# 10183308/popsift

Measured on AMD Instinct MI355X. Metric: Mpix/s SIFT extract on 1920x1080 (keypoints+descriptors), higher is better.
Workload: dtype f32; 1 GPU; 1920x1080 u8 grayscale, default popsift::Config (2x upscale, 9 octaves, 3 levels, PopSift mode, loop descriptor, RootSift); distinct_images_per_gpu=16, contexts_per_gpu=3, images_per_launch=16

## Files before the change

popsift_amd/csrc/ctx.hip:

```cpp
#include <hip/hip_runtime.h>

#include <algorithm>
#include <atomic>
#include <cmath>
#include <cstdarg>
#include <cstddef>
#include <cstdio>
#include <cstdlib>
#include <cstring>
#include <new>
#include <type_traits>
#include <vector>

#include "devfeatures.h"
#include "kernels.h"
#include "sift_types.h"
#include "trace.h"

using namespace popsift_hip;

namespace {

constexpr int PITCH_ALIGN = 64;
constexpr int PROFILE_REPS = 4;

template <int N>
struct GaussRows {
    float filter[N * PS_GA];
    int   span[N];
    float sigma[N];
};

struct EventPair {
    hipEvent_t a, b;
    double     bytes;
    bool       big;
};

template <class T, size_t PER = 1>
struct DevBuf {
    T*     p = nullptr;
    size_t cap = 0;
    hipError_t release()
    {
        const hipError_t e = p ? hipFree(p) : hipSuccess;
        if (e == hipSuccess) {
            p = nullptr;
            cap = 0;
        }
        return e;
    }
};

}

struct ImageSlot {
    DevBuf<char> input;
    void*        h_input = nullptr;
    size_t       h_input_cap = 0;
    DevBuf<float>       arena;
    DevBuf<InitExt>     iext;
    DevBuf<InitExt>     iext2;
    DevBuf<FilterState> fstate;
    DevBuf<int>         fhist;
    DevBuf<InitExt>     otmp;
    DevBuf<int>         orows;
    DevBuf<Ext>         ext;
    DevBuf<float, PS_ORI_NBINS> ohist;
    DevBuf<popsift_hip_feature> feats;
    DevBuf<float, 128> desc;
    DevBuf<int>        map;
    DevBuf<float2>     rot;
    DevBuf<DescRec>    drec;
    DevBuf<int2>       cand;
    DevBuf<int>        partial;
    DevBuf<int>        ovf;
    bool               sized = false;
    DevBuf<popsift_hip_feature> alt_feats;
    DevBuf<float, 128>          alt_desc;
    bool moved = false;
    DevBuf<uint8_t, 128> desc_u8;
    bool u8_read = false;
    DevBuf<popsift_hip_frame>   frames;
    popsift_hip_frame*          h_frames = nullptr;
    DevBuf<int>                 fcounts, perm, inv;
    DevBuf<popsift_hip_feature> lfeats;
    int n_frames = 0;

    size_t desc_cap() const { return std::min({desc.cap, map.cap, rot.cap, drec.cap}); }

    void release()
    {
        auto each = [](auto&... b) { ((void)b.release(), ...); };
        each(input, arena, iext, iext2, fstate, fhist, otmp, orows, ext, ohist, feats, desc, map, rot, drec, cand, partial, ovf, alt_feats,
             alt_desc, desc_u8, frames, fcounts, perm, inv, lfeats);
        if (h_input) (void)hipHostFree(h_input);
        if (h_frames) (void)hipHostFree(h_frames);
    }
};

struct popsift_hip_ctx {
    int                device = 0;
    popsift_hip_params p{};
    int                levels = 3, L = 6;
    GaussRows<POPSIFT_HIP_MAX_LEVELS> tab{};
    GaussRows<POPSIFT_HIP_MAX_LEVELS> abs0{};
    float*             d_abs0 = nullptr;
    int                direct_path = 0;
    GaussRows<POPSIFT_HIP_MAX_OCTAVES> dd{};
    float*             d_dd = nullptr;
    int                scale_path = 0;
    SiftConsts         sc{};
    hipStream_t        stream = nullptr;
    hipEvent_t         ev_begin = nullptr, ev_end = nullptr;
    hipEvent_t         ev_stage[POPSIFT_HIP_STAGE_COUNT + 1] = {};

    int  in_w = 0, in_h = 0;
    int  frozen_octaves = -1;
    bool have_image = false, finished = false;
    bool batch_ok = false;
    int  nb = 1;
    bool describe = false;
    int  ori_given = 0;
    int  frames_max = 0;

    ImageSlot slot[PS_MAX_BATCH];
    BatchDesc bd{};
    PyrDesc   pd{};
    int       kp_waves = 65536;
    int       det_qcap = 1 << 30;
    int       desc_rows = 1 << 30;
    int       desc_list = 1 << 30;
    BlurTune  blur_tune{0, 0};
    int       order_coarse = 0;
    int       pyr_tail = 0;
    int       cand_cap_init = 1 << 20;
    bool      cand_cap_user = false;
    int       ohist_cap_init = 0;
    int       desc_cap_init = 0;
    size_t    ext_cap = 0;
    int       cand_cap = 0, desc_cap = 0;
    size_t    ohist_cap = 0;
    hipStream_t copy_stream = nullptr;
    hipEvent_t  ev_u8 = nullptr;
    bool     copy_pending = false;
    unsigned long submit_seq = 0, copy_seq = 0;
    Counters* d_ct = nullptr;
    Counters* h_ct = nullptr;
    PyrDesc*  d_pd = nullptr;
    PyrDesc*  h_pd = nullptr;
    int       n_feat[PS_MAX_BATCH] = {}, n_desc[PS_MAX_BATCH] = {};

    int                    fail_alloc_in = 0;
    int                    profile = 0;
    std::vector<EventPair> blur_events;
    size_t                 blur_events_used = 0;
    popsift_hip_report     rep{};

    char err[256] = {0};
};

namespace {

int fail(popsift_hip_ctx* c, int code, const char* fmt, ...)
{
    if (c) {
        va_list ap;
        va_start(ap, fmt);
        vsnprintf(c->err, sizeof(c->err), fmt, ap);
        va_end(ap);
    }
    return code;
}

#define HIP_TRY(c, call)                                                                              \
    do {                                                                                              \
        hipError_t e__ = (call);                                                                      \
// ... 102 lines not shown

void plan_dims(const popsift_hip_params& p, int w, int h, int octaves_cfg, int* n_oct, int* bw, int* bh)
{
    const float scaleFactor = 1.0f / powf(2.0f, -p.upscale_factor);
    int         oct = octaves_cfg;
    if (oct < 0) oct = std::max(int(floorf(logf((float)std::min(w, h)) / logf(2.0f)) - 3.0f + scaleFactor), 1);
    oct = std::min(oct, PS_MAX_OCT);
    *n_oct = oct;
    *bw = (int)ceilf(w * scaleFactor);
    *bh = (int)ceilf(h * scaleFactor);
}

const char* plan_pyramid(const popsift_hip_params& p, int levels, int L, int octaves_cfg, int w, int h, PyrDesc* out,
                         size_t* arena_floats, int* base_w, int* base_h)
{
    int n_oct, bw, bh;
    memset(out, 0, sizeof(*out));
    *arena_floats = 0;
    plan_dims(p, w, h, octaves_cfg, &n_oct, &bw, &bh);
    *base_w = bw;
    *base_h = bh;
    if (bw < 1 || bh < 1) return "scaled image is empty";
    if (bw > 32767 || bh > 32767) return "scaled image exceeds 32767 pixels per side";
    PyrDesc& pd = *out;
    size_t   total = 0;
    pd.n_oct = n_oct;
    pd.levels = levels;
    pd.L = L;
    pd.dog_fly = p.store_dog ? 0 : 1;
    int ow = bw, oh = bh, tiles = 0;
    for (int o = 0; o < n_oct; o++) {
        OctDesc& od = pd.o[o];
        od.w = ow;
        od.h = oh;
        od.pitch = (ow + PITCH_ALIGN - 1) / PITCH_ALIGN * PITCH_ALIGN;
        od.plane_stride = (int64_t)od.pitch * oh;
        od.tile_begin = tiles;
        tiles += extrema_units(ow, oh);
        od.data_off = (int64_t)total;
        total += (size_t)od.plane_stride * (size_t)L;
        if (!pd.dog_fly) {
            od.dog_off = (int64_t)total;
            total += (size_t)od.plane_stride * (size_t)(L - 1);
        }
        ow = (int)ceilf(ow / 2.0f);
        oh = (int)ceilf(oh / 2.0f);
    }
    if (pd.dog_fly) {
        for (int o = 0; o < n_oct; o++) pd.o[o].dog_off = (int64_t)total;
        total += (size_t)pd.o[0].plane_stride;
    }
    pd.total_tiles = tiles;
    *arena_floats = total;
    if (total * sizeof(float) >= ((size_t)1 << 32)) return "pyramid arena of 4 GiB or more: the image is too large";
    return nullptr;
}

hipError_t ctx_malloc(popsift_hip_ctx* c, void** p, size_t bytes)
{
    if (c->fail_alloc_in > 0 && --c->fail_alloc_in == 0) {
        *p = nullptr;
        return hipErrorOutOfMemory;
    }
    return hipMalloc(p, bytes);
}

template <class T, size_t PER>
int grow(popsift_hip_ctx* c, DevBuf<T, PER>& b, size_t need)
{
    if (need <= b.cap) return 0;
    HIP_TRY(c, b.release());
    HIP_TRY(c, ctx_malloc(c, (void**)&b.p, need * PER * sizeof(T)));
    b.cap = need;
    return 0;
}

void refresh_caps(popsift_hip_ctx* c)
{
    size_t cand = 1 << 30, desc = 1 << 30, hist = (size_t)1 << 40;
    for (int k = 0; k < c->nb; k++) {
        const ImageSlot& s = c->slot[k];
        cand = std::min(cand, s.cand.cap);
        desc = std::min(desc, s.desc_cap());
        hist = std::min(hist, s.ohist.cap);
        Slot& v = c->bd.s[k];
        v.arena = s.arena.p;
        v.ct = c->d_ct + k;
        v.cand = s.cand.p;
        v.ovf = s.ovf.p;
        v.iext = s.iext.p;
        v.iext2 = s.iext2.p;
        v.fstate = s.fstate.p;
        v.fhist = s.fhist.p;
        v.ohist = s.ohist.p;
        v.ext = s.ext.p;
        v.partial = s.partial.p;
        v.map = s.map.p;
        v.rot = s.rot.p;
        v.drec = s.drec.p;
        v.feats = s.feats.p;
        v.desc = s.desc.p;
    }
    c->cand_cap = (int)cand;
    c->desc_cap = (int)desc;
    c->ohist_cap = hist;
}

int slot_desc_cap(popsift_hip_ctx* c, ImageSlot& s, size_t need)
{
    if (need <= s.desc_cap()) return 0;
    HIP_TRY(c, s.desc.release());
    HIP_TRY(c, s.map.release());
    HIP_TRY(c, s.rot.release());
    HIP_TRY(c, s.drec.release());
    if (int rc = grow(c, s.desc, need)) return rc;
    if (int rc = grow(c, s.map, need)) return rc;
    if (int rc = grow(c, s.rot, need)) return rc;
    return grow(c, s.drec, need);
}

template <typename F>
int ensure_cap(popsift_hip_ctx* c, F grow_slot)
{
    int rc = 0;
    for (int k = 0; k < c->nb && !rc; k++) rc = grow_slot(c->slot[k]);
    refresh_caps(c);
    return rc;
}

int prepare_geometry(popsift_hip_ctx* c, int w, int h, int nb)
{
    const bool same = c->have_image && w == c->in_w && h == c->in_h && c->pd.n_oct > 0;
    PyrDesc    pd = c->pd;
    int        bw = c->rep.base_w, bh = c->rep.base_h;
    size_t     total = 0;
    if (!same) {
        PyrDesc plan;
        if (const char* why = plan_pyramid(c->p, c->levels, c->L, c->frozen_octaves, w, h, &plan, &total, &bw, &bh))
            return fail(c, POPSIFT_HIP_ERR_INVALID, why);
        if (c->sc.filter_max > 0 && !filter_supported(plan.n_oct, c->sc.max_extrema, c->sc.grid_size))
            return fail(c, POPSIFT_HIP_ERR_INVALID, "grid filter: grid size > 64 or octaves * max_extrema >= 2^25");
        c->frozen_octaves = plan.n_oct;

        c->in_w = c->in_h = 0;
        c->have_image = false;
        c->pd.n_oct = 0;
        c->ext_cap = 0;
        for (int k = 0; k < PS_MAX_BATCH; k++) c->slot[k].sized = false;

        pd = plan;
    } else {
        const OctDesc& last = pd.o[pd.n_oct - 1];
        total = pd.dog_fly ? (size_t)pd.o[0].dog_off + (size_t)pd.o[0].plane_stride
                           : (size_t)last.dog_off + (size_t)last.plane_stride * (size_t)(c->L - 1);
    }
    const size_t need_ext = (size_t)pd.n_oct * (size_t)c->sc.max_extrema;
    for (int k = 0; k < nb; k++) {
        ImageSlot& s = c->slot[k];
        if (s.sized) continue;
        if (int rc = grow(c, s.arena, total)) return rc;
        if (int rc = grow(c, s.iext, need_ext)) return rc;
        if (int rc = grow(c, s.ext, need_ext)) return rc;
        if (int rc = grow(c, s.feats, need_ext)) return rc;
        if (c->sc.filter_max > 0) {
            if (int rc = grow(c, s.iext2, need_ext)) return rc;
            if (int rc = grow(c, s.fstate, 1)) return rc;
            if (int rc = grow(c, s.fhist, filter_hist_bytes(c->sc.grid_size) / sizeof(int))) return rc;
        }
        if (c->p.feature_order == POPSIFT_HIP_ORDER_RASTER) {
            if (int rc = grow(c, s.otmp, need_ext)) return rc;
            if (int rc = grow(c, s.orows, order_rows(pd))) return rc;
        }
        if (int rc = grow(c, s.partial, (need_ext / scan_chunk() + 2) * scan_partials_per_chunk())) return rc;
        const int desc0 = c->desc_cap_init > 0 ? c->desc_cap_init
                                               : std::max(2 * c->sc.max_extrema, c->sc.max_extrema + c->sc.max_extrema / 4);
        if (int rc = slot_desc_cap(c, s, std::max(desc0, c->desc_cap))) return rc;
        int cand0 = std::max(c->cand_cap_init, DET_SUBQ);
        if (!c->cand_cap_user) {
            double px = 0;
            for (int o = 0; o < pd.n_oct; o++) px += (double)pd.o[o].w * pd.o[o].h;
            cand0 = std::max(cand0, (int)std::min(px / 8.0, 64.0 * 1024 * 1024));
        }
        if (int rc = grow(c, s.cand, std::max(cand0, c->cand_cap))) return rc;
        if (int rc = grow(c, s.ohist, std::max(c->ohist_cap_init > 0 ? (size_t)c->ohist_cap_init
                                                                      : std::min(need_ext, (size_t)2 * c->sc.max_extrema),
                                               c->slot[0].sized ? c->ohist_cap : (size_t)0)))
            return rc;
        if (int rc = grow(c, s.ovf, (size_t)pd.total_tiles + 1)) return rc;
        s.sized = true;
    }
    c->ext_cap = need_ext;
    if (!same) {
        *c->h_pd = pd;
        HIP_TRY(c, hipMemcpyAsync(c->d_pd, c->h_pd, sizeof(PyrDesc), hipMemcpyHostToDevice, c->stream));
        c->pd = pd;
        c->in_w = w;
        c->in_h = h;
        c->rep.num_octaves = pd.n_oct;
        c->rep.base_w = bw;
        c->rep.base_h = bh;
        double px = 0;
        for (int o = 0; o < pd.n_oct; o++) px += (double)pd.o[o].w * pd.o[o].h;
        c->rep.pyramid_pixels = px;
    }
    return 0;
}

template <typename F>
int timed_launch(popsift_hip_ctx* c, double alg_bytes, const char* what, F launch, bool big = false)
{
    if (c->profile == 1) {
        if (c->blur_events_used == c->blur_events.size()) {
            EventPair ep;
            HIP_TRY(c, hipEventCreate(&ep.a));
            HIP_TRY(c, hipEventCreate(&ep.b));
            c->blur_events.push_back(ep);
        }
        EventPair& ep = c->blur_events[c->blur_events_used++];
        ep.bytes = alg_bytes * c->nb;
        ep.big = big;
        HIP_TRY(c, hipEventRecord(ep.a, c->stream));
        for (int rep = 0; rep < PROFILE_REPS; rep++) HIP_TRY(c, launch());
        HIP_TRY(c, hipEventRecord(ep.b, c->stream));
    } else {
        HIP_TRY(c, launch());
        SYNC_CHK(c, what);
    }
    (void)what;
    return 0;
}

int blur_launch(popsift_hip_ctx* c, const BlurArgs& a, int mode, int span, int tile_h, double alg_bytes)
{
    return timed_launch(
        c, alg_bytes, "k_blur_tile", [&] { return launch_blur(a, c->bd, c->nb, mode, span, tile_h, c->stream, c->blur_tune); },
        mode == 0 && tile_h == 64);
}

template <typename A>
void set_plane(A& a, const OctDesc& od, int tile_h)
{
    a.w = od.w;
    a.h = od.h;
    a.pitch = od.pitch;
    a.tiles_x = (od.w + blur_tile_w() - 1) / blur_tile_w();
    a.tiles_y = (od.h + tile_h - 1) / tile_h;
}

BlurArgs level_args(const popsift_hip_ctx* c, int o, int level)
{
    const PyrDesc& pd = c->pd;
    const OctDesc& od = pd.o[o];
    BlurArgs       a{};
    set_plane(a, od, blur_tile_h(od.w, od.h));
    memcpy(a.taps.g, &c->tab.filter[level * PS_GA], sizeof(a.taps.g));
    a.dst_off = od.data_off + level * od.plane_stride;
    a.src_off = od.data_off + (level - 1) * od.plane_stride;
    a.dog_off = pd.dog_fly ? -1 : od.dog_off + (level - 1) * od.plane_stride;
    a.next0_off = (level == pd.L - 3 && o + 1 < pd.n_oct) ? pd.o[o + 1].data_off : -1;
    a.next_pitch = (o + 1 < pd.n_oct) ? pd.o[o + 1].pitch : 0;
    return a;
}

float input_shift(const popsift_hip_ctx* c)
{
    if (c->p.sift_mode == POPSIFT_HIP_SIFT_POPSIFT || c->p.sift_mode == POPSIFT_HIP_SIFT_VLFEAT)
        return 0.5f * powf(2.0f, c->p.upscale_factor - 0);
// ... 356 lines not shown
        const size_t bytes = (size_t)w * h * esz;
        if (int rc = grow(c, s.input, bytes)) return rc;
        if (where == 2) {
            HIP_TRY(c, hipMemcpy2DAsync(s.input.p, (size_t)w * esz, imgs[k], (size_t)pitch * esz, (size_t)w * esz, (size_t)h,
                                        hipMemcpyHostToDevice, c->stream));
        } else {
            if (bytes > s.h_input_cap) {
                if (s.h_input) HIP_TRY(c, hipHostFree(s.h_input));
                s.h_input = nullptr;
                s.h_input_cap = 0;
                HIP_TRY(c, hipHostMalloc(&s.h_input, bytes, hipHostMallocDefault));
                s.h_input_cap = bytes;
            }
            for (int y = 0; y < h; y++)
                memcpy((char*)s.h_input + (size_t)y * w * esz, (const char*)imgs[k] + (size_t)y * pitch * esz, (size_t)w * esz);
            HIP_TRY(c, hipMemcpyAsync(s.input.p, s.h_input, bytes, hipMemcpyHostToDevice, c->stream));
        }
        c->bd.s[k].input = s.input.p;
        dpitch = w;
    }
    if (where != 1) aligned4 = (dpitch & 3) == 0;
    c->describe = da != nullptr;
    c->ori_given = da && da->ori_mode == POPSIFT_HIP_ORI_GIVEN;
    c->frames_max = 0;
    for (int k = 0; k < nb && da; k++) {
        ImageSlot& s = c->slot[k];
        if (int rc = prepare_frames(c, s)) return rc;
        const int nf = da->n_frames[k];
        s.n_frames = nf;
        c->frames_max = std::max(c->frames_max, nf);
        if (nf > 0) {
            memcpy(s.h_frames, da->frames[k], (size_t)nf * sizeof(popsift_hip_frame));
            HIP_TRY(c, hipMemcpyAsync(s.frames.p, s.h_frames, (size_t)nf * sizeof(popsift_hip_frame), hipMemcpyHostToDevice, c->stream));
        }
    }
    c->blur_events_used = 0;
    HIP_TRY(c, hipEventRecord(c->ev_begin, c->stream));
    if (c->profile == 2) HIP_TRY(c, hipEventRecord(c->ev_stage[POPSIFT_HIP_STAGE_PYRAMID], c->stream));
    if (int rc = enqueue_pyramid(c, is_f32, dpitch, aligned4)) return rc;
    if (int rc = da ? enqueue_describe_stages(c, true) : enqueue_keypoint_stages(c, true)) return rc;
    HIP_TRY(c, hipEventRecord(c->ev_end, c->stream));
    c->have_image = true;
    c->finished = false;
    c->batch_ok = true;
    c->submit_seq++;
    for (ImageSlot& sl : c->slot) sl.moved = false;
    return 0;
}

int finish(popsift_hip_ctx* c)
{
    if (!c->have_image || !c->batch_ok) return fail(c, POPSIFT_HIP_ERR_STATE, c->have_image ? "the last submit failed" : "no image submitted");
    if (c->finished) return 0;
    POPSIFT_RANGE("popsift_hip: wait");
    HIP_TRY(c, hipSetDevice(c->device));
    bool rerun = false, fits = false;
    for (int attempt = 0; attempt < 8; attempt++) {
        HIP_TRY(c, hipStreamSynchronize(c->stream));
        int  ori_max = 0, qmax = 0;
        long ext_max = 0;
        for (int k = 0; k < c->nb; k++) {
            const Counters& h = c->h_ct[k];
            ori_max = std::max(ori_max, h.ori_total);
            for (int q = 0; q < DET_SUBQ; q++) qmax = std::max(qmax, h.qcnt[q].n);
            long ext_sum = 0;
            for (int o = 0; o < c->pd.n_oct; o++) ext_sum += std::min(h.ext_ct[o], c->sc.max_extrema);
            ext_max = std::max(ext_max, ext_sum);
        }
        const bool desc_short = ori_max > c->desc_cap;
        const bool cand_short = qmax > c->cand_cap / DET_SUBQ;
        const bool hist_short = (size_t)ext_max > c->ohist_cap && !c->ori_given;
        if (!desc_short && !cand_short && !hist_short) {
            fits = true;
            break;
        }
        if (desc_short)
            if (int rc = ensure_cap(c, [&](ImageSlot& s) { return slot_desc_cap(c, s, ori_max + ori_max / 8 + 1024); }))
                return rc;
        if (cand_short)
            if (int rc = ensure_cap(c, [&](ImageSlot& s) { return grow(c, s.cand, DET_SUBQ * (qmax + qmax / 8 + 64)); }))
                return rc;
        if (hist_short) {
            const size_t need = (size_t)ext_max + (size_t)ext_max / 8 + 1024;
            if (int rc = ensure_cap(c, [&](ImageSlot& s) { return grow(c, s.ohist, need); })) return rc;
        }
        if (int rc = c->describe ? enqueue_describe_stages(c) : enqueue_keypoint_stages(c)) return rc;
        HIP_TRY(c, hipEventRecord(c->ev_end, c->stream));
        rerun = true;
    }
    if (!fits) return fail(c, POPSIFT_HIP_ERR_DEVICE, "the keypoint buffers still do not fit after 8 grow-and-rerun rounds");
    popsift_hip_report& r = c->rep;
    for (int k = 0; k < c->nb; k++) {
        c->n_feat[k] = c->describe ? c->slot[k].n_frames : c->h_ct[k].ext_total;
        c->n_desc[k] = std::min(c->h_ct[k].ori_total, c->desc_cap);
    }
    Counters& h0 = c->h_ct[0];
    int       next = h0.ori_total;
    for (int o = PS_MAX_OCT - 1; o >= 0; o--) {
        if (h0.ext_ct[o] > 0) {
            h0.ori_ct[o] = next - h0.ori_ps[o];
            next = h0.ori_ps[o];
        } else {
            h0.ori_ct[o] = 0;
            h0.ori_ps[o] = next;
        }
    }
    for (int o = 0; o < PS_MAX_OCT; o++) {
        r.ext_ct[o] = h0.ext_ct[o];
        r.ori_ct[o] = h0.ori_ct[o];
    }
    r.ext_total = c->h_ct[0].ext_total;
    r.ori_total = c->n_desc[0];
    float ms = 0.0f;
    if (hipEventElapsedTime(&ms, c->ev_begin, c->ev_end) == hipSuccess) r.ms_device = ms;
    for (int k = 0; k < 8; k++) r.ms_stage[k] = 0.0f;
    if (c->profile == 2 && !rerun)
        for (int k = 0; k < POPSIFT_HIP_STAGE_COUNT; k++) {
            float t = 0.0f;
            if (hipEventElapsedTime(&t, c->ev_stage[k], c->ev_stage[k + 1]) == hipSuccess) r.ms_stage[k] = t;
        }
    r.ms_blur = 0.0f;
    r.blur_launches = 0;
    r.blur_alg_bytes = 0.0;
    r.ms_big = 0.0f;
    r.big_launches = 0;
    r.big_alg_bytes = 0.0;
    for (size_t i = 0; i < c->blur_events_used; i++) {
        float t = 0.0f;
        if (hipEventElapsedTime(&t, c->blur_events[i].a, c->blur_events[i].b) == hipSuccess) {
            t /= (float)PROFILE_REPS;
            r.ms_blur += t;
            r.blur_launches++;
            r.blur_alg_bytes += c->blur_events[i].bytes;
            if (c->blur_events[i].big) {
                r.ms_big += t;
                r.big_launches++;
                r.big_alg_bytes += c->blur_events[i].bytes;
            }
        }
    }
    c->finished = true;
    return 0;
}

int drain_copy(popsift_hip_ctx* c)
{
    if (!c->copy_pending) return 0;
    c->copy_pending = false;
    HIP_TRY(c, hipStreamSynchronize(c->copy_stream));
    return 0;
}

int results_here(popsift_hip_ctx* c, int k = 0)
{
    if (int rc = finish(c)) return rc;
    if (k < 0 || k >= c->nb) return fail(c, POPSIFT_HIP_ERR_INVALID, "the batch has %d images", c->nb);
    if (c->slot[k].moved)
        return fail(c, POPSIFT_HIP_ERR_STATE, "the results of this image were handed to popsift_hip_fetch_begin");
    return 0;
}

int slot_u8_ready(popsift_hip_ctx* c, ImageSlot& sl)
{
    if (sl.u8_read && c->copy_pending) HIP_TRY(c, hipStreamSynchronize(c->copy_stream));
    sl.u8_read = false;
    return grow(c, sl.desc_u8, std::max<size_t>(sl.desc_cap(), 1));
}
// ... 1278 lines not shown
```

popsift_amd/csrc/keypoint.hip:

```cpp
#include <hip/hip_runtime.h>

#include "kernels.h"
#include "sift_types.h"

namespace popsift_hip {
namespace {

constexpr float F_PI = 3.14159265358979323846f;
constexpr float F_PI2 = 2.0f * 3.14159265358979323846f;
constexpr float            ORI_WINFACTOR = 1.5f;
constexpr float            DESC_MAGNIFY = 3.0f;

typedef unsigned long long fix64;
__device__ __forceinline__ fix64 to_fix(float w) { return (fix64)(unsigned int)(w * 1048576.0f); }
__device__ __forceinline__ float from_fix(fix64 v) { return (float)((double)v * (1.0 / 1048576.0)); }


__device__ __forceinline__ void wave_lds_sync()
{
    __builtin_amdgcn_fence(__ATOMIC_SEQ_CST, "wavefront");
    __builtin_amdgcn_wave_barrier();
}

__device__ __forceinline__ int wave_incl_scan(int v)
// ... 120 lines not shown
    r = (ay > ax) ? 1.5707963267948966f - r : r;
    r = (x < 0.0f) ? 3.14159265358979323846f - r : r;
    return (y < 0.0f) ? -r : r;
}

__device__ __forceinline__ void sincos_cr(float ang, float& s, float& c)
{
    const double x = (double)ang;
    const double q = rint(x * 0.63661977236758134308);
    double       r = fma(-q, 1.57079632679489655800e+00, x);
    r = fma(-q, 6.12323399573676603587e-17, r);
    const double z = r * r;
    double       ps = 2.81145725434552075980e-15;
    ps = fma(ps, z, -7.64716373181981647590e-13);
    ps = fma(ps, z, 1.60590438368216145994e-10);
    ps = fma(ps, z, -2.50521083854417187751e-08);
    ps = fma(ps, z, 2.75573192239858906526e-06);
    ps = fma(ps, z, -1.98412698412698412698e-04);
    ps = fma(ps, z, 8.33333333333333333333e-03);
    ps = fma(ps, z, -1.66666666666666666667e-01);
    const double sr = fma(ps * z, r, r);
    double       pc = -1.56192069685862264622e-16;
    pc = fma(pc, z, 4.77947733238738529744e-14);
    pc = fma(pc, z, -1.14707455977297247139e-11);
    pc = fma(pc, z, 2.08767569878680989792e-09);
    pc = fma(pc, z, -2.75573192239858906526e-07);
    pc = fma(pc, z, 2.48015873015873015873e-05);
    pc = fma(pc, z, -1.38888888888888888889e-03);
    pc = fma(pc, z, 4.16666666666666666667e-02);
    pc = fma(pc, z, -0.5);
    const double cr = fma(pc, z, 1.0);
    const int    n = (int)q & 3;
    const double sd = (n & 1) ? cr : sr, cd = (n & 1) ? sr : cr;
    s = (float)((n & 2) ? -sd : sd);
    c = (float)(((n + 1) & 2) ? -cd : cd);
}

__device__ __forceinline__ float octants(float t, float x, float y, float ax, float ay)
{
    const unsigned int sgn = 0x80000000u;
    const float a = __uint_as_float(__float_as_uint(1.0f - t) ^ (__float_as_uint(ax - ay) & sgn));
    const float b = __uint_as_float(__float_as_uint(1.0f + a) ^ (__float_as_uint(x) & sgn));
    return copysignf(2.0f - b, y);
}

__device__ __forceinline__ float atan2_bins(float y, float x)
{
    const float ax = fabsf(x), ay = fabsf(y);
    const float mx = fmaxf(fmaxf(ax, ay), 1e-30f), mn = fminf(ax, ay);
    const float r = mn * __builtin_amdgcn_rcpf(mx);
    const float s = r * r;
    float       p = fmaf(-0.01492126751691103f, s, 0.06703268736600876f);
    p = fmaf(p, s, -0.14823880791664124f);
    p = fmaf(p, s, 0.24642325937747955f);
    p = fmaf(p, s, -0.42350852489471436f);
    p = fmaf(p, s, 1.2732105255126953f);
    return octants(p * r, x, y, ax, ay);
}

__device__ __forceinline__ float atan2_bins9(float y, float x)
{
    const float ax = fabsf(x), ay = fabsf(y);
    const float mx = fmaxf(fmaxf(ax, ay), 1e-30f), mn = fminf(ax, ay);
    const float r = mn * __builtin_amdgcn_rcpf(mx);
    const float s = r * r;
    float       p = fmaf(0.026540832594037056f, s, -0.1084246039390564f);
    p = fmaf(p, s, 0.22938621044158936f);
    p = fmaf(p, s, -0.4205572307109833f);
    p = fmaf(p, s, 1.2730693817138672f);
    return octants(p * r, x, y, ax, ay);
}

typedef float v2f __attribute__((ext_vector_type(2)));
typedef __attribute__((address_space(3))) fix64 lds_fix64;
typedef __attribute__((address_space(3))) unsigned int lds_u32;
typedef __attribute__((address_space(3))) short lds_i16;
typedef __attribute__((address_space(3))) unsigned long long lds_u64;

#ifndef KP_NW
#define KP_NW 1
#endif
constexpr int ORI_COPIES = 4;

__global__ __launch_bounds__(64 * KP_NW) void k_orientation(const PyrDesc* __restrict__ pdp, BatchDesc bd, SiftConsts sc,
                                                     int filtered, int hist_cap)
{
    const float* __restrict__   arena = bd.s[blockIdx.y].arena;
    Counters* __restrict__      ct = bd.s[blockIdx.y].ct;
    const InitExt* __restrict__ iext = filtered ? bd.s[blockIdx.y].iext2 : bd.s[blockIdx.y].iext;
    float* __restrict__         ohist = bd.s[blockIdx.y].ohist;
    const int n_oct = pdp->n_oct, L = pdp->L;
    constexpr int    NB = PS_ORI_NBINS + 2;
    __shared__ fix64 s_hist[KP_NW][ORI_COPIES][NB];
    const int        wave = threadIdx.x >> 6, lane = threadIdx.x & 63;
    fix64*           hall = &s_hist[wave][0][0];
    fix64*           hist = s_hist[wave][lane & (ORI_COPIES - 1)];

    __shared__ int ps[PS_MAX_OCT + 1];
    if (threadIdx.x == 0) ext_prefix(ct, sc, n_oct, ps);
    __syncthreads();
    const int total = min(ps[n_oct], hist_cap);

    for (XcdSlice sl = xcd_slice<KP_NW>(); sl.more(total); sl.s += sl.step) {
        const int g = sl.index();
        if (g >= total) continue;
        int o = 0;
        while (o + 1 < n_oct && g >= ps[o + 1]) o++;
        o = uniform(o);
        const InitExt  ie = iext[(size_t)o * sc.max_extrema + (g - uniform(ps[o]))];
        const OctDesc* od = &pdp->o[o];
        const int      w = uniform(od->w), h = uniform(od->h), pitch = uniform(od->pitch);
        const int      lvl = uniform(min(max(ie.lpos, 0), L - 1));
        const float*   layer = arena + uniform64(od->data_off + lvl * od->plane_stride);

        for (int k = lane; k < ORI_COPIES * NB; k += 64) hall[k] = 0ull;
        wave_lds_sync();

        const float x = uniformf(ie.xpos), y = uniformf(ie.ypos), sig = uniformf(ie.sigma);
        const float sigw = ORI_WINFACTOR * sig;
        const int   rad = (int)roundf(3.0f * sigw);
        const float factor2 = (-0.5f / (sigw * sigw)) * 1.4426950408889634f;
        const int   sq_thres = rad * rad;
        const int   xmin = max(1, (int)roundf(x) - rad);
        const int   xmax = min(w - 2, (int)roundf(x) + rad);
        const int   ymin = max(1, (int)roundf(y) - rad);
        const int   ymax = min(h - 2, (int)roundf(y) + rad);
        const int   wx = xmax - xmin + 1;
        const int   hy = ymax - ymin + 1;
#ifdef ORI_PROBE_NOLOOP
        const int   loops = 0;
#else
        const int   loops = (wx > 0 && hy > 0) ? wx * hy : 0;
#endif
        const float inv_wx = __builtin_amdgcn_rcpf((float)max(wx, 1));
        const float wxf = (float)wx, xminf = (float)xmin, yminf = (float)ymin, pitch4f = (float)(4 * pitch);
        const float* corner = layer + (size_t)(ymin * pitch + xmin);

        auto coord = [&](int i, float& fx, float& fy, unsigned int& off) {
            const float fi = (float)i;
            const float frow = floorf((fi + 0.5f) * inv_wx);
            const float fcol = fmaf(-frow, wxf, fi);
            fx = fcol + xminf;
            fy = frow + yminf;
            off = (unsigned int)fmaf(frow, pitch4f, fcol * 4.0f);
        };
        auto bin = [&](float fx, float fy, float gdx, float gdy, bool live) {
            const float dx = fx - x;
            const float dy = fy - y;
            const float sq_dist = truncf(dx * dx + dy * dy);
            if (live && sq_dist <= (float)sq_thres) {
                const float wfix = __builtin_amdgcn_sqrtf(fmaf(gdx, gdx, gdy * gdy)) * __builtin_amdgcn_exp2f(fmaf(sq_dist, factor2, 20.0f));
                float fb = fmaf(atan2_bins(gdy, gdx), (float)PS_ORI_NBINS / 8.0f, (float)PS_ORI_NBINS / 2.0f);
                if (fabsf((fb - floorf(fb)) - 0.5f) < 1e-4f) fb = (float)PS_ORI_NBINS * (atan2_acc(gdy, gdx) + F_PI) / F_PI2;
                int bidx;
                asm("v_cvt_rpi_i32_f32 %0, %1" : "=v"(bidx) : "v"(fb));
                atomicAdd(&hist[bidx], (fix64)(unsigned int)wfix);
            }
        };
        float        xa = 0.0f, ya = 0.0f, xb = 0.0f, yb = 0.0f;
        unsigned int oa = 0, ob = 0;
        float        a0 = 0.0f, a1 = 0.0f, a2 = 0.0f, a3 = 0.0f, b0 = 0.0f, b1 = 0.0f, b2 = 0.0f, b3 = 0.0f;
        const Taps   taps(corner, pitch);
        if (loops > 0) {
            coord(min(lane, loops - 1), xa, ya, oa);
            taps.load_b(oa, a0, a1, a2, a3);
        }
        for (int i = lane; i < loops; i += 128) {
            coord(min(i + 64, loops - 1), xb, yb, ob);
            taps.load_b(ob, b0, b1, b2, b3);
            bin(xa, ya, a0 - a1, a2 - a3, true);
            coord(min(i + 128, loops - 1), xa, ya, oa);
            taps.load_b(oa, a0, a1, a2, a3);
            bin(xb, yb, b0 - b1, b2 - b3, i + 64 < loops);
        }
        wave_lds_sync();

        if (lane < PS_ORI_NBINS) {
            fix64 acc = 0ull;
#pragma unroll
            for (int k = 0; k < ORI_COPIES; k++) acc += hall[k * NB + lane] + (lane == 0 ? hall[k * NB + PS_ORI_NBINS] : 0ull);
            ohist[(size_t)g * PS_ORI_NBINS + lane] = from_fix(acc);
        }
        wave_lds_sync();
    }
}

__device__ __forceinline__ float quad_from_prev(float v)
{
    return __int_as_float(__builtin_amdgcn_update_dpp(0, __float_as_int(v), 0x93, 0xf, 0xf, false));
}
__device__ __forceinline__ float quad_from_next(float v)
{
    return __int_as_float(__builtin_amdgcn_update_dpp(0, __float_as_int(v), 0x39, 0xf, 0xf, false));
}
template <int CTRL>
__device__ __forceinline__ int quad_xchg(int v)
{
    return __builtin_amdgcn_update_dpp(0, v, CTRL, 0xf, 0xf, false);
}
__device__ __forceinline__ float div3(float x)
{
    const float r = 0.333333343267440796f;
    const float q = x * r;
    return fmaf(fmaf(-3.0f, q, x), r, q);
}

__device__ __forceinline__ int ori_peaks_quad(const float* __restrict__ hsrc, int j, bool have, float* angle_out)
{
    constexpr int N = PS_ORI_NBINS, M = N / 4;
    float         h[M], t[M];
#pragma unroll
    for (int b = 0; b < M; b++) h[b] = have ? hsrc[M * j + b] : 0.0f;
#pragma unroll
    for (int pass = 0; pass < 3; pass++) {
        {
            const float lft = quad_from_prev(h[M - 1]), rgt = quad_from_next(h[0]);
#pragma unroll
            for (int b = 0; b < M; b++) t[b] = div3(((b == 0 ? lft : h[b - 1]) + h[b]) + (b == M - 1 ? rgt : h[b + 1]));
        }
        {
            const float lft = quad_from_prev(t[M - 1]), rgt = quad_from_next(t[0]);
#pragma unroll
            for (int b = 0; b < M; b++) h[b] = div3(((b == 0 ? lft : t[b - 1]) + t[b]) + (b == M - 1 ? rgt : t[b + 1]));
        }
    }
    float refined[M], yval[M];
    {
        const float lft = quad_from_prev(h[M - 1]), rgt = quad_from_next(h[0]);
#pragma unroll
        for (int b = 0; b < M; b++) {
            const int   bin = M * j + b;
            const int   prev = (bin == 0) ? N - 1 : bin - 1;
            const float hp = (b == 0) ? lft : h[b - 1], hv = h[b], hn = (b == M - 1) ? rgt : h[b + 1];
            bool        predicate = hv > fmaxf(hp, hn);
            const float num = predicate ? 3.0f * hp - 4.0f * hv + 1.0f * hn : 0.0f;
            const float denB = predicate ? 2.0f * (hp - 2.0f * hv + hn) : 1.0f;
            const float newbin = num / denB;
            predicate = (predicate && newbin >= 0.0f && newbin <= 2.0f);
            refined[b] = predicate ? prev + newbin : -1.0f;
            yval[b] = predicate ? -(num * num) / (4.0f * denB) + hp : -INFINITY;
        }
    }
    unsigned int used = 0u;
    float        best0 = 0.0f;
    int          angles = 0;
#pragma unroll
    for (int k = 0; k < POPSIFT_HIP_ORI_MAX; k++) {
        float bv = 0.0f, br = -1.0f;
        int   bi = -1;
#pragma unroll
        for (int b = 0; b < M; b++) {
            const bool take = !((used >> b) & 1u) && (bi < 0 || yval[b] > bv);
            bv = take ? yval[b] : bv;
            br = take ? refined[b] : br;
            bi = take ? M * j + b : bi;
        }
        {
// ... 733 lines not shown
                    }
                }
            } else
            for (int p = lane; p < 1600; p += 64) {
                const int   newy = p / 40, newx = p - newy * 40;
                const float stepx = stepbase + 0.125f * (float)newx;
                const float stepy = stepbase + 0.125f * (float)newy;
                const float ptx = cos_t * stepx + -sin_t * stepy;
                const float pty = cos_t * stepy + sin_t * stepx;
                const float px = x + ptx * SBP, py = y + pty * SBP;
                const float dxv = tex_linear(layer, width, height, pitch, px + cos_t, py + sin_t) -
                                  tex_linear(layer, width, height, pitch, px - cos_t, py - sin_t);
                const float dyv = tex_linear(layer, width, height, pitch, px - sin_t, py + cos_t) -
                                  tex_linear(layer, width, height, pitch, px + sin_t, py - cos_t);
                const float mod = __builtin_amdgcn_sqrtf(dxv * dxv + dyv * dyv);
                float       th = atan2_acc(dyv, dxv);
                th += (th < 0.0f ? F_PI2 : 0.0f);
                const float tth = th * M_4RPI;
                const float ffo = floorf(tth);
                const float do0 = tth - ffo;
                const int   b0 = (int)ffo & 7;
                const float ww = __expf(-0.125f * (stepx * stepx + stepy * stepy)) * mod * fscale;
                const float a1 = do0 * ww, a0 = ww - a1;
#pragma unroll
                for (int jy = 0; jy < 2; jy++) {
                    const int cy = (newy >> 3) - jy;
                    if (cy < 0 || cy > 3) continue;
                    const float wy = 1.0f - fabsf(-1.0f + 1.0f / 16.0f + 0.125f * (float)(newy - 8 * cy));
#pragma unroll
                    for (int jx = 0; jx < 2; jx++) {
                        const int cx = (newx >> 3) - jx;
                        if (cx < 0 || cx > 3) continue;
                        const float wx = 1.0f - fabsf(-1.0f + 1.0f / 16.0f + 0.125f * (float)(newx - 8 * cx));
                        const float wgt = wx * wy;
                        const unsigned int lo = (unsigned int)fmaf(a0, wgt, 0.5f);
                        const unsigned int hi = (unsigned int)fmaf(a1, wgt, 0.5f);
                        atomicAdd(&hist[((((cy << 2) + cx) << 3)) + b0], ((fix64)hi << 32) | lo);
                    }
                }
            }
        }
        wave_lds_sync();

        fix64     a0 = 0ull, a1 = 0ull;
        const int prevw = (lane & ~7) | ((lane + 7) & 7);
#pragma unroll
        for (int k = 0; k < DCOPY; k++) {
            a0 += (hall[k * 128 + lane] & 0xffffffffull) + (hall[k * 128 + prevw] >> 32);
            a1 += (hall[k * 128 + lane + 64] & 0xffffffffull) + (hall[k * 128 + prevw + 64] >> 32);
        }
        float v0 = (float)a0 * (1.0f / (float)(1 << FBITS)), v1 = (float)a1 * (1.0f / (float)(1 << FBITS));

        if (sc.norm_mode == POPSIFT_HIP_NORM_ROOTSIFT) {
            float sum = v0 + v1;
            sum = wave_allsum(sum);
            v0 = scalbnf(sqrtf(v0 / sum), sc.norm_multi);
            v1 = scalbnf(sqrtf(v1 / sum), sc.norm_multi);
        } else {
            float sq = v0 * v0 + v1 * v1;
            sq = wave_allsum(sq);
            const float norm = sqrtf(sq);
            v0 = fminf(v0, 0.2f * norm);
            v1 = fminf(v1, 0.2f * norm);
            sq = v0 * v0 + v1 * v1;
            sq = wave_allsum(sq);
            float rn = 1.0f / sqrtf(sq);
            rn = scalbnf(rn, sc.norm_multi);
            v0 = v0 * rn;
            v1 = v1 * rn;
        }
        desc[(size_t)d * 128 + lane] = v0;
        desc[(size_t)d * 128 + 64 + lane] = v1;
        wave_lds_sync();
    }
}



}

hipError_t launch_orientation(const PyrDesc* pd, const BatchDesc& bd, int nb, const SiftConsts& sc, bool filtered, int hist_cap,
                              int blocks, hipStream_t s)
{
    hipLaunchKernelGGL(k_orientation, dim3(blocks / KP_NW, nb), dim3(64 * KP_NW), 0, s, pd, bd, sc, filtered ? 1 : 0, hist_cap);
    return hipGetLastError();
}

hipError_t launch_scan(const PyrDesc* pd, const BatchDesc& bd, int nb, const SiftConsts& sc, bool filtered, int hist_cap,
                       int n_chunks, int desc_cap, hipStream_t s)
{
    hipLaunchKernelGGL(k_scan_local, dim3(std::min(n_chunks * SCAN_SUB, 512 * SCAN_SUB), nb), dim3(SCAN_LT), 0, s, pd, sc, bd,
                       filtered ? 1 : 0, hist_cap);
    hipLaunchKernelGGL(k_scan_apply, dim3(std::min(n_chunks, 1024), nb), dim3(256), 0, s, pd, sc, bd,
                       sc.desc_mode == POPSIFT_HIP_DESC_LOOP ? 1 : 0, desc_cap);
    return hipGetLastError();
}

hipError_t launch_scan_apply(const PyrDesc* pd, const BatchDesc& bd, int nb, const SiftConsts& sc, int n_chunks, int desc_cap,
                             hipStream_t s)
{
    hipLaunchKernelGGL(k_scan_apply, dim3(std::min(n_chunks, 1024), nb), dim3(256), 0, s, pd, sc, bd,
                       sc.desc_mode == POPSIFT_HIP_DESC_LOOP ? 1 : 0, desc_cap);
    return hipGetLastError();
}

int scan_chunk() { return SCAN_CHUNK; }
int scan_partials_per_chunk() { return SCAN_SUB; }

hipError_t launch_descriptors(const PyrDesc* pd, const BatchDesc& bd, int nb, const SiftConsts& sc, int desc_cap, int blocks,
                              hipStream_t s)
{
    if (sc.desc_mode == POPSIFT_HIP_DESC_NOTILE || sc.desc_mode == POPSIFT_HIP_DESC_IGRID)
        hipLaunchKernelGGL(k_descriptor_notile<false>, dim3(blocks / 4, nb), dim3(256), 0, s, pd, bd, sc, desc_cap);
    else if (sc.desc_mode == POPSIFT_HIP_DESC_ILOOP)
        hipLaunchKernelGGL(k_descriptor_notile<true>, dim3(blocks / 4, nb), dim3(256), 0, s, pd, bd, sc, desc_cap);
    else if (sc.desc_mode == POPSIFT_HIP_DESC_GRID)
        hipLaunchKernelGGL(k_descriptor_grid, dim3(blocks / 4, nb), dim3(256), 0, s, pd, bd, sc, desc_cap);
    else
        hipLaunchKernelGGL(k_descriptor, dim3(blocks / KP_NW, nb), dim3(64 * KP_NW), 0, s, bd, sc, desc_cap);
    return hipGetLastError();
}


}
```

popsift_amd/csrc/sift_types.h:

```cpp
#pragma once
#include <stdint.h>

#include <hip/hip_vector_types.h>

#include "../../include/popsift_hip.h"

#define PS_MAX_OCT POPSIFT_HIP_MAX_OCTAVES
#define PS_MAX_PLANES (POPSIFT_HIP_MAX_LEVELS + 3)
#define PS_GA POPSIFT_HIP_GAUSS_ALIGN
#define PS_ORI_NBINS 36

struct OctDesc {
    float*  data;
    float*  dog;
    int64_t data_off;
    int64_t dog_off;
    int64_t plane_stride;
    int     w, h, pitch;
    int     tile_begin;
};

struct PyrDesc {
    int     n_oct;
    int     levels;
    int     L;
    int     total_tiles;
    int     dog_fly;
    int     pad_;
    OctDesc o[PS_MAX_OCT];
};

struct SiftConsts {
    float sigma0, sigma_k, edge_limit, threshold;
    int   max_extrema, norm_multi, norm_mode, sift_mode;
    int   grid_size;
    int   up_fac_int;
    int   desc_mode;
    int   det_qcap;
    int   filter_max;
    int   filter_mode;
    int   desc_rows;
    int   desc_list;
};

struct InitExt {
    float xpos, ypos;
    int   lpos;
    float sigma;
    int   cell;
};

struct Ext {
    float xpos, ypos;
    int   lpos;
    float sigma;
    int   octave;
    int   num_ori;
    int   idx_ori;
    float orientation[POPSIFT_HIP_ORI_MAX];
};

struct DescRec {
    float        x, y;
    float        crsbp, srsbp;
    float        ang_bins;
    float        inv_c;
    unsigned int xymin, xymax;
    unsigned int off_lo, off_hi;
    unsigned int misc;
    float        inv_s;
};

static_assert(sizeof(DescRec) == 48, "three 16-byte loads");

struct Counters {
    int ext_ct[PS_MAX_OCT];
    int ori_ct[PS_MAX_OCT];
    int ext_ps[PS_MAX_OCT];
    int ori_ps[PS_MAX_OCT];
    int ext_total;
    int ori_total;
    int pad[2];
    struct {
        int n;
        int pad[31];
    } qcnt[64];
};
#define DET_SUBQ 64

#define PS_MAX_BATCH POPSIFT_HIP_MAX_BATCH
struct FilterState;
struct Slot {
    float*               arena;
    Counters*            ct;
    const void*          input;
    int2*                cand;
    int*                 ovf;
    InitExt*             iext;
    InitExt*             iext2;
    FilterState*         fstate;
    int*                 fhist;
    float*               ohist;
    Ext*                 ext;
    int*                 partial;
    int*                 map;
    float2*              rot;
    DescRec*             drec;
    popsift_hip_feature* feats;
    float*               desc;
};
struct BatchDesc {
    Slot s[PS_MAX_BATCH];
};

#define FILTER_MAX_CELLS 4096
struct FilterState {
    int                active;
    int                newlimit;
    int                pad[2];
    int                new_ct[PS_MAX_OCT];
    int                cell_count[FILTER_MAX_CELLS];
    int                cell_limit[FILTER_MAX_CELLS];
    int                remaining[FILTER_MAX_CELLS];
    int                cell_mode[FILTER_MAX_CELLS];
    unsigned long long prefix[FILTER_MAX_CELLS];
};

struct FrameSlot {
    const popsift_hip_frame* frames;
    int*                     counts;
    int*                     perm;
    int*                     inv;
    popsift_hip_feature*     lfeats;
    int                      n;
    int                      pad_;
};
struct FrameBatch {
    FrameSlot s[PS_MAX_BATCH];
};

struct OrderSlot {
    InitExt*        list;
    InitExt*        tmp;
    int*            rows;
    const Counters* ct;
};
struct OrderBatch {
    OrderSlot s[PS_MAX_BATCH];
};
struct OrderArgs {
    int n_oct, coarse, max_extrema;
    int chunks;
    int rows_total;
    int row_base[PS_MAX_OCT];
    int rows[PS_MAX_OCT];
};
```

Measured before the change: 3874 Mpix/s.

## Precompute per-keypoint orientation records in a prep kernel and restructure histogram loop

Adds a k_ori_prep kernel that computes each extremum's orientation window parameters (bounds, gaussian factor, threshold, corner offset) once per thread and stores them as 48-byte OriRec records. The orientation kernel then reads each record with three scalar 16-byte loads instead of doing the octave search, InitExt fetch and setup math per wave. It also splits the software-pipelined sample loop into a steady-state body with no bounds clamps and an explicit tail. This trades an extra kernel launch and an extra buffer write/read for less serial scalar setup in the wave-per-keypoint loop.

```diff
diff --git a/popsift_amd/csrc/ctx.hip b/popsift_amd/csrc/ctx.hip
--- a/popsift_amd/csrc/ctx.hip
+++ b/popsift_amd/csrc/ctx.hip
@@ -67,6 +67,7 @@
     DevBuf<int>         orows;
     DevBuf<Ext>         ext;
     DevBuf<float, PS_ORI_NBINS> ohist;
+    DevBuf<OriRec>              orec;
     DevBuf<popsift_hip_feature> feats;
     DevBuf<float, 128> desc;
     DevBuf<int>        map;
@@ -88,11 +89,12 @@
     int n_frames = 0;
 
     size_t desc_cap() const { return std::min({desc.cap, map.cap, rot.cap, drec.cap}); }
+    size_t hist_cap() const { return std::min(ohist.cap, orec.cap); }
 
     void release()
     {
         auto each = [](auto&... b) { ((void)b.release(), ...); };
-        each(input, arena, iext, iext2, fstate, fhist, otmp, orows, ext, ohist, feats, desc, map, rot, drec, cand, partial, ovf, alt_feats,
+        each(input, arena, iext, iext2, fstate, fhist, otmp, orows, ext, ohist, orec, feats, desc, map, rot, drec, cand, partial, ovf, alt_feats,
              alt_desc, desc_u8, frames, fcounts, perm, inv, lfeats);
         if (h_input) (void)hipHostFree(h_input);
         if (h_frames) (void)hipHostFree(h_frames);
@@ -361,7 +363,7 @@
         const ImageSlot& s = c->slot[k];
         cand = std::min(cand, s.cand.cap);
         desc = std::min(desc, s.desc_cap());
-        hist = std::min(hist, s.ohist.cap);
+        hist = std::min(hist, s.hist_cap());
         Slot& v = c->bd.s[k];
         v.arena = s.arena.p;
         v.ct = c->d_ct + k;
@@ -372,6 +374,7 @@
         v.fstate = s.fstate.p;
         v.fhist = s.fhist.p;
         v.ohist = s.ohist.p;
+        v.orec = s.orec.p;
         v.ext = s.ext.p;
         v.partial = s.partial.p;
         v.map = s.map.p;
@@ -396,6 +399,15 @@
     if (int rc = grow(c, s.map, need)) return rc;
     if (int rc = grow(c, s.rot, need)) return rc;
     return grow(c, s.drec, need);
+}
+
+int slot_hist_cap(popsift_hip_ctx* c, ImageSlot& s, size_t need)
+{
+    if (need <= s.hist_cap()) return 0;
+    HIP_TRY(c, s.ohist.release());
+    HIP_TRY(c, s.orec.release());
+    if (int rc = grow(c, s.ohist, need)) return rc;
+    return grow(c, s.orec, need);
 }
 
 template <typename F>
@@ -461,7 +473,7 @@
             cand0 = std::max(cand0, (int)std::min(px / 8.0, 64.0 * 1024 * 1024));
         }
         if (int rc = grow(c, s.cand, std::max(cand0, c->cand_cap))) return rc;
-        if (int rc = grow(c, s.ohist, std::max(c->ohist_cap_init > 0 ? (size_t)c->ohist_cap_init
+        if (int rc = slot_hist_cap(c, s, std::max(c->ohist_cap_init > 0 ? (size_t)c->ohist_cap_init
                                                                       : std::min(need_ext, (size_t)2 * c->sc.max_extrema),
                                                c->slot[0].sized ? c->ohist_cap : (size_t)0)))
             return rc;
@@ -984,7 +996,7 @@
                 return rc;
         if (hist_short) {
             const size_t need = (size_t)ext_max + (size_t)ext_max / 8 + 1024;
-            if (int rc = ensure_cap(c, [&](ImageSlot& s) { return grow(c, s.ohist, need); })) return rc;
+            if (int rc = ensure_cap(c, [&](ImageSlot& s) { return slot_hist_cap(c, s, need); })) return rc;
         }
         if (int rc = c->describe ? enqueue_describe_stages(c) : enqueue_keypoint_stages(c)) return rc;
         HIP_TRY(c, hipEventRecord(c->ev_end, c->stream));
diff --git a/popsift_amd/csrc/keypoint.hip b/popsift_amd/csrc/keypoint.hip
--- a/popsift_amd/csrc/keypoint.hip
+++ b/popsift_amd/csrc/keypoint.hip
@@ -226,41 +226,29 @@
 #endif
 constexpr int ORI_COPIES = 4;
 
-__global__ __launch_bounds__(64 * KP_NW) void k_orientation(const PyrDesc* __restrict__ pdp, BatchDesc bd, SiftConsts sc,
-                                                     int filtered, int hist_cap)
-{
-    const float* __restrict__   arena = bd.s[blockIdx.y].arena;
-    Counters* __restrict__      ct = bd.s[blockIdx.y].ct;
-    const InitExt* __restrict__ iext = filtered ? bd.s[blockIdx.y].iext2 : bd.s[blockIdx.y].iext;
-    float* __restrict__         ohist = bd.s[blockIdx.y].ohist;
+
+__global__ __launch_bounds__(256) void k_ori_prep(const PyrDesc* __restrict__ pdp, BatchDesc bd, SiftConsts sc, int filtered,
+                                                  int hist_cap)
+{
+    const Counters* __restrict__ ct = bd.s[blockIdx.y].ct;
+    const InitExt* __restrict__  iext = filtered ? bd.s[blockIdx.y].iext2 : bd.s[blockIdx.y].iext;
+    OriRec* __restrict__         orec = bd.s[blockIdx.y].orec;
     const int n_oct = pdp->n_oct, L = pdp->L;
-    constexpr int    NB = PS_ORI_NBINS + 2;
-    __shared__ fix64 s_hist[KP_NW][ORI_COPIES][NB];
-    const int        wave = threadIdx.x >> 6, lane = threadIdx.x & 63;
-    fix64*           hall = &s_hist[wave][0][0];
-    fix64*           hist = s_hist[wave][lane & (ORI_COPIES - 1)];
-
     __shared__ int ps[PS_MAX_OCT + 1];
     if (threadIdx.x == 0) ext_prefix(ct, sc, n_oct, ps);
     __syncthreads();
     const int total = min(ps[n_oct], hist_cap);
 
-    for (XcdSlice sl = xcd_slice<KP_NW>(); sl.more(total); sl.s += sl.step) {
-        const int g = sl.index();
-        if (g >= total) continue;
+    for (int g = blockIdx.x * blockDim.x + threadIdx.x; g < total; g += gridDim.x * blockDim.x) {
         int o = 0;
         while (o + 1 < n_oct && g >= ps[o + 1]) o++;
-        o = uniform(o);
-        const InitExt  ie = iext[(size_t)o * sc.max_extrema + (g - uniform(ps[o]))];
+        const InitExt  ie = iext[(size_t)o * sc.max_extrema + (g - ps[o])];
         const OctDesc* od = &pdp->o[o];
-        const int      w = uniform(od->w), h = uniform(od->h), pitch = uniform(od->pitch);
-        const int      lvl = uniform(min(max(ie.lpos, 0), L - 1));
-        const float*   layer = arena + uniform64(od->data_off + lvl * od->plane_stride);
-
-        for (int k = lane; k < ORI_COPIES * NB; k += 64) hall[k] = 0ull;
-        wave_lds_sync();
-
-        const float x = uniformf(ie.xpos), y = uniformf(ie.ypos), sig = uniformf(ie.sigma);
+        const int      w = od->w, h = od->h, pitch = od->pitch;
+        const int      lvl = min(max(ie.lpos, 0), L - 1);
+        const long long layer = od->data_off + lvl * od->plane_stride;
+
+        const float x = ie.xpos, y = ie.ypos, sig = ie.sigma;
         const float sigw = ORI_WINFACTOR * sig;
         const int   rad = (int)roundf(3.0f * sigw);
         const float factor2 = (-0.5f / (sigw * sigw)) * 1.4426950408889634f;
@@ -271,14 +259,67 @@
         const int   ymax = min(h - 2, (int)roundf(y) + rad);
         const int   wx = xmax - xmin + 1;
         const int   hy = ymax - ymin + 1;
+        const int   loops = (wx > 0 && hy > 0) ? wx * hy : 0;
+        const float inv_wx = __builtin_amdgcn_rcpf((float)max(wx, 1));
+        const long long corner = layer + (long long)(ymin * pitch + xmin);
+
+        OriRec r;
+        r.x = x;
+        r.y = y;
+        r.factor2 = factor2;
+        r.sq_thres = (float)sq_thres;
+        r.xminf = (float)xmin;
+        r.yminf = (float)ymin;
+        r.wxf = (float)wx;
+        r.inv_wx = inv_wx;
+        r.loops = loops;
+        r.pitch = pitch;
+        r.off_lo = (unsigned int)((unsigned long long)corner & 0xffffffffull);
+        r.off_hi = (unsigned int)((unsigned long long)corner >> 32);
+        orec[g] = r;
+    }
+}
+
+typedef unsigned int u32x4 __attribute__((ext_vector_type(4)));
+
+__global__ __launch_bounds__(64 * KP_NW) void k_orientation(const PyrDesc* __restrict__ pdp, BatchDesc bd, SiftConsts sc,
+                                                     int hist_cap)
+{
+    const int n_oct = pdp->n_oct;
+    const float* __restrict__ arena = bd.s[blockIdx.y].arena;
+    float* __restrict__       ohist = bd.s[blockIdx.y].ohist;
+    const __attribute__((address_space(4))) u32x4* orec = (const __attribute__((address_space(4))) u32x4*)bd.s[blockIdx.y].orec;
+    constexpr int    NB = PS_ORI_NBINS + 2;
+    __shared__ fix64 s_hist[KP_NW][ORI_COPIES][NB];
+    const int        wave = threadIdx.x >> 6, lane = threadIdx.x & 63;
+    fix64*           hall = &s_hist[wave][0][0];
+    fix64*           hist = s_hist[wave][lane & (ORI_COPIES - 1)];
+
+    const __attribute__((address_space(4))) Counters* ct = (const __attribute__((address_space(4))) Counters*)bd.s[blockIdx.y].ct;
+    int total = 0;
+    for (int o = 0; o < n_oct; o++) total += min(ct->ext_ct[o], sc.max_extrema);
+    total = min(total, hist_cap);
+
+    for (XcdSlice sl = xcd_slice<KP_NW>(); sl.more(total); sl.s += sl.step) {
+        const int g = uniform(sl.index());
+        if (g >= total) continue;
+        const u32x4 q0 = orec[3 * (size_t)g], q1 = orec[3 * (size_t)g + 1], q2 = orec[3 * (size_t)g + 2];
+
+        for (int k = lane; k < ORI_COPIES * NB; k += 64) hall[k] = 0ull;
+        wave_lds_sync();
+
+        const float x = __uint_as_float(q0.x), y = __uint_as_float(q0.y), factor2 = __uint_as_float(q0.z);
+        const float sq_thres = __uint_as_float(q0.w);
+        const float xminf = __uint_as_float(q1.x), yminf = __uint_as_float(q1.y);
+        const float wxf = __uint_as_float(q1.z), inv_wx = __uint_as_float(q1.w);
 #ifdef ORI_PROBE_NOLOOP
         const int   loops = 0;
 #else
-        const int   loops = (wx > 0 && hy > 0) ? wx * hy : 0;
+        const int   loops = (int)q2.x;
 #endif
-        const float inv_wx = __builtin_amdgcn_rcpf((float)max(wx, 1));
-        const float wxf = (float)wx, xminf = (float)xmin, yminf = (float)ymin, pitch4f = (float)(4 * pitch);
-        const float* corner = layer + (size_t)(ymin * pitch + xmin);
+        const int   pitch = (int)q2.y;
+        const float pitch4f = (float)(4 * pitch);
+        const float* corner = arena + (long long)(((unsigned long long)q2.w << 32) | q2.z);
 
         auto coord = [&](int i, float& fx, float& fy, unsigned int& off) {
             const float fi = (float)i;
@@ -292,7 +333,7 @@
             const float dx = fx - x;
             const float dy = fy - y;
             const float sq_dist = truncf(dx * dx + dy * dy);
-            if (live && sq_dist <= (float)sq_thres) {
+            if (live && sq_dist <= sq_thres) {
                 const float wfix = __builtin_amdgcn_sqrtf(fmaf(gdx, gdx, gdy * gdy)) * __builtin_amdgcn_exp2f(fmaf(sq_dist, factor2, 20.0f));
                 float fb = fmaf(atan2_bins(gdy, gdx), (float)PS_ORI_NBINS / 8.0f, (float)PS_ORI_NBINS / 2.0f);
                 if (fabsf((fb - floorf(fb)) - 0.5f) < 1e-4f) fb = (float)PS_ORI_NBINS * (atan2_acc(gdy, gdx) + F_PI) / F_PI2;
@@ -309,14 +350,27 @@
             coord(min(lane, loops - 1), xa, ya, oa);
             taps.load_b(oa, a0, a1, a2, a3);
         }
-        for (int i = lane; i < loops; i += 128) {
+        int base = 0, i = lane;
+        for (; base + 192 <= loops; base += 128, i += 128) {
+            coord(i + 64, xb, yb, ob);
+            taps.load_b(ob, b0, b1, b2, b3);
+            bin(xa, ya, a0 - a1, a2 - a3, true);
+            coord(i + 128, xa, ya, oa);
+            taps.load_b(oa, a0, a1, a2, a3);
+            bin(xb, yb, b0 - b1, b2 - b3, true);
+        }
+        const int rem = (loops - base + 63) >> 6;
+        if (rem >= 2) {
             coord(min(i + 64, loops - 1), xb, yb, ob);
             taps.load_b(ob, b0, b1, b2, b3);
-            bin(xa, ya, a0 - a1, a2 - a3, true);
+        }
+        if (rem >= 1) bin(xa, ya, a0 - a1, a2 - a3, i < loops);
+        if (rem == 3) {
             coord(min(i + 128, loops - 1), xa, ya, oa);
             taps.load_b(oa, a0, a1, a2, a3);
-            bin(xb, yb, b0 - b1, b2 - b3, i + 64 < loops);
-        }
+        }
+        if (rem >= 2) bin(xb, yb, b0 - b1, b2 - b3, i + 64 < loops);
+        if (rem == 3) bin(xa, ya, a0 - a1, a2 - a3, i + 128 < loops);
         wave_lds_sync();
 
         if (lane < PS_ORI_NBINS) {
@@ -1216,7 +1270,9 @@
 hipError_t launch_orientation(const PyrDesc* pd, const BatchDesc& bd, int nb, const SiftConsts& sc, bool filtered, int hist_cap,
                               int blocks, hipStream_t s)
 {
-    hipLaunchKernelGGL(k_orientation, dim3(blocks / KP_NW, nb), dim3(64 * KP_NW), 0, s, pd, bd, sc, filtered ? 1 : 0, hist_cap);
+    const int prep = std::min(std::max((hist_cap + 255) / 256, 1), 1024);
+    hipLaunchKernelGGL(k_ori_prep, dim3(prep, nb), dim3(256), 0, s, pd, bd, sc, filtered ? 1 : 0, hist_cap);
+    hipLaunchKernelGGL(k_orientation, dim3(blocks / KP_NW, nb), dim3(64 * KP_NW), 0, s, pd, bd, sc, hist_cap);
     return hipGetLastError();
 }
 
diff --git a/popsift_amd/csrc/sift_types.h b/popsift_amd/csrc/sift_types.h
--- a/popsift_amd/csrc/sift_types.h
+++ b/popsift_amd/csrc/sift_types.h
@@ -73,6 +73,19 @@
 
 static_assert(sizeof(DescRec) == 48, "three 16-byte loads");
 
+struct alignas(16) OriRec {
+    float        x, y;
+    float        factor2;
+    float        sq_thres;
+    float        xminf, yminf;
+    float        wxf, inv_wx;
+    int          loops;
+    int          pitch;
+    unsigned int off_lo, off_hi;
+};
+
+static_assert(sizeof(OriRec) == 48 && alignof(OriRec) == 16, "three 16-byte loads");
+
 struct Counters {
     int ext_ct[PS_MAX_OCT];
     int ori_ct[PS_MAX_OCT];
@@ -101,6 +114,7 @@
     FilterState*         fstate;
     int*                 fhist;
     float*               ohist;
+    OriRec*              orec;
     Ext*                 ext;
     int*                 partial;
     int*                 map;
```

Measured after the change: 3835 Mpix/s. 1.0% lower.
